# pgvector/pgvector

Hardware: AMD Instinct MI355X
Metric: QPS @ recall@10 (IVFFlat, 1M x 1536d) (higher is better)
Workload: dtype f32

## Files before the change

### pgvector_amd/csrc/kernels_query.hip

```cpp
#include "pgv_device.h"
#include "pgv_select.h"

#include <type_traits>

namespace pgv {

namespace {

constexpr int kQThreads = kSelThreads;
constexpr int kQWaves = kQThreads / kWave;
constexpr int kMaxBatchLists = 256;
constexpr int kHeadCap = 1024;

template <typename T, int METRIC, int NCH> struct WholeRows {
    Raw16 q[NCH];
    __device__ __forceinline__ void load_query(const char *qp, int lane) {
#pragma unroll
        for (int c = 0; c < NCH; c++) q[c] = load16(qp + ((size_t)c * kWave + lane) * sizeof(Raw16));
    }
    __device__ __forceinline__ float pair(const char *a, const char *b, int lane) const {
        Raw16 ra[NCH], rb[NCH];
#pragma unroll
        for (int c = 0; c < NCH; c++) ra[c] = load16(a + ((size_t)c * kWave + lane) * sizeof(Raw16));
#pragma unroll
// ... 727 lines not shown
    run_geometry(ctx, g, ix->nlists, &per, &grid);
    const int kp = pow2_at_least(max_probes);
    PGV_TRY(dispatch_metric(ix->metric, ix->dtype, [&](auto *tp, auto mc) {
        using T = std::remove_pointer_t<decltype(tp)>;
        constexpr int M = decltype(mc)::value;
        return dispatch_nch<T, M>(g, [&](auto nc) {
            constexpr int NCH = decltype(nc)::value;
            hipLaunchKernelGGL((mq_rank_kernel<T, M, NCH>), dim3(grid, nq), dim3(kQThreads), 0, ctx->stream,
                               static_cast<const char *>(ix->centers), ix->nlists, g.nvec, g.lpr_log2,
                               static_cast<const char *>(q_dev), cdist, cd_stride, per);
            PGV_HIP(hipGetLastError());
            return PGV_OK;
        });
    }));
    hipLaunchKernelGGL(mq_lists_kernel, dim3(nq), dim3(kQThreads), kQueryLds, ctx->stream, cdist, cd_stride, ix->nlists,
                       max_probes, kp, out_lists, out_dist);
    PGV_HIP(hipGetLastError());
    return PGV_OK;
}

int launch_multi_scan(pgv_ctx *ctx, const pgv_index *ix, const void *q_dev, int nq, const int32_t *probe_lists, int nprobes,
                      int64_t rows_bound, float *seg, int64_t seg_stride, int k, float *out_dist, int64_t *out_slot,
                      uint64_t *out_tid) {
    const RowGeom &g = ix->geom;
    int per, grid;
    run_geometry(ctx, g, rows_bound, &per, &grid);
    const int cap = (ctx->num_cus * 8 + nq - 1) / nq;
    if (grid > cap) grid = cap < 1 ? 1 : cap;
    PGV_TRY(dispatch_metric(ix->metric, ix->dtype, [&](auto *tp, auto mc) {
        using T = std::remove_pointer_t<decltype(tp)>;
        constexpr int M = decltype(mc)::value;
        return dispatch_nch<T, M>(g, [&](auto nc) {
            constexpr int NCH = decltype(nc)::value;
            hipLaunchKernelGGL((mq_scan_kernel<T, M, NCH>), dim3(grid, nq), dim3(kQThreads), 0, ctx->stream,
                               static_cast<const char *>(ix->vectors), ix->list_offsets, probe_lists, nprobes, g.nvec,
                               g.lpr_log2, static_cast<const char *>(q_dev), seg, seg_stride, per);
            PGV_HIP(hipGetLastError());
            return PGV_OK;
        });
    }));
    double *stats = (ctx->profiling && ctx->stats_dev.p) ? ctx->stats_dev.as<double>() : nullptr;
    hipLaunchKernelGGL(mq_head_kernel, dim3(nq), dim3(kQThreads), kQueryLds, ctx->stream, seg, seg_stride, ix->list_offsets,
                       ix->tids, probe_lists, nprobes, k, pow2_at_least(k), out_dist, out_slot, out_tid, stats);
    PGV_HIP(hipGetLastError());
    return PGV_OK;
}

namespace {
struct ApproxScratch {
    float *cand_val = nullptr;
    int64_t *cand_pos = nullptr;
    int32_t *flags = nullptr;
    int carve(DBuf &buf, int nq, int kprime) {
        const size_t nk = (size_t)nq * kprime;
        const size_t a1 = (sizeof(float) * nk + 15) & ~(size_t)15, a2 = a1 + sizeof(int64_t) * nk;
        PGV_TRY(buf.ensure(a2 + sizeof(int32_t) * (2 * (size_t)nq + 1)));
        cand_val = buf.as<float>();
        cand_pos = reinterpret_cast<int64_t *>(buf.as<char>() + a1);
        flags = reinterpret_cast<int32_t *>(buf.as<char>() + a2);
        return PGV_OK;
    }
};
}

int launch_exact_tail(pgv_ctx *ctx, const ExactTail &t, DBuf &scratch) {
    if (t.nq <= 0) return PGV_OK;
    const ExactRows &xr = t.rows;
    const bool dense = t.dense();
    if (dense ? (t.fixed_len <= 0 || t.probe_off || t.seg_start || t.probes != 0)
              : (t.fixed_len != 0 || !t.probe_off || !t.seg_start || t.probes < 1))
        PGV_FAIL(PGV_ERR_ARG, "exact tail: a list plan or one dense run");
    if (t.kprime > kRecheckCap || t.k > t.kprime)
        PGV_FAIL(PGV_ERR_ARG, "exact tail: k' = %d outside k..%d", t.kprime, kRecheckCap);
    if (t.pair_t && xr.dtype != PGV_F32) PGV_FAIL(PGV_ERR_ARG, "exact tail: pair terms are for fp32 rows");
    static_assert(kWide >= kRecheckCap, "k <= k' <= kWide: batch_fix_kernel's emit");
    if (t.emit.cnt && !(dense && t.pair_t && t.out_i32 && t.emit.probe_off && t.emit.seg_len && t.emit.list_off))
        PGV_FAIL(PGV_ERR_ARG, "exact tail: the plan is counted where the pair terms are written");
    ApproxScratch sc;
    PGV_TRY(sc.carve(scratch, t.nq, t.kprime));
    const int64_t *cand_slot = dense ? sc.cand_pos : nullptr;
    const int64_t *seg_start = dense ? nullptr : t.seg_start;
    const int64_t fixed_len = dense ? t.fixed_len : 0;
    PGV_TRY(launch_topk_segments(ctx, t.approx, seg_start, t.nq, fixed_len, t.kprime, sc.cand_val, sc.cand_pos,
                                 sc.flags + t.nq, t.emit.cnt, t.emit.cnt ? 2 * (int)fixed_len : 0));
#define PGV_RECHECK(T, DOT)                                                                                          \
    hipLaunchKernelGGL((batch_recheck_kernel<T, DOT>), dim3(t.nq), dim3(kQThreads), 0, ctx->stream,                   \
                       static_cast<const char *>(xr.vectors), xr.tids, xr.geom.nvec, xr.geom.lpr_log2,                \
                       static_cast<const char *>(t.queries), t.kprime, t.k, sc.cand_val, sc.cand_pos, cand_slot,      \
                       xr.list_offsets, t.probe_lists, t.probe_off, t.probes, seg_start, fixed_len, xr.norm_max,      \
                       t.bound, t.eps_add, t.nq, t.out_dist, t.out_slot, t.out_tid, t.out_i32, sc.flags, t.pair_t,    \
                       t.emit)
    if (t.pair_t)
        PGV_RECHECK(float, true);
    else if (xr.dtype == PGV_F32)
        PGV_RECHECK(float, false);
    else
        PGV_RECHECK(__half, false);
#undef PGV_RECHECK
    PGV_HIP(hipGetLastError());
    double *stats = (ctx->profiling && ctx->stats_dev.p) ? ctx->stats_dev.as<double>() : nullptr;
    int kp = 2;
    while (kp < t.k) kp <<= 1;
    const int cap = kp > kFastCap ? kp : kFastCap;
    const size_t lds = (size_t)cap * 8 + sizeof(SelShared);
    const int grid = t.nq < ctx->num_cus ? t.nq : ctx->num_cus;
#define PGV_FIX(T)                                                                                                    \
    hipLaunchKernelGGL(batch_fix_kernel<T>, dim3(grid), dim3(kQThreads), lds, ctx->stream,                            \
                       static_cast<const char *>(xr.vectors), xr.list_offsets, xr.tids, xr.geom.nvec,                 \
                       xr.geom.lpr_log2, static_cast<const char *>(t.queries), t.probe_lists, t.probe_off, t.probes,  \
                       seg_start, fixed_len, sc.flags, t.nq, t.approx, t.k, kp, cap, xr.norm_max, t.bound, t.eps_add, \
                       ctx->no_widen ? 0 : 1, t.out_dist, t.out_slot, t.out_tid, t.out_i32, stats, t.pair_t, t.emit)
    if (xr.dtype == PGV_F32)
        PGV_FIX(float);
    else
        PGV_FIX(__half);
#undef PGV_FIX
    PGV_HIP(hipGetLastError());
    return PGV_OK;
}

}
```

### pgvector_amd/csrc/kernels_select.hip

```cpp
#include "pgv_device.h"
#include "pgv_select.h"

namespace pgv {

namespace {


__global__ void plan_count_kernel(const int32_t *__restrict__ probe_lists,
                                  const int64_t *__restrict__ list_off, int nq, int probes,
                                  int *__restrict__ cnt, int64_t *__restrict__ probe_off,
                                  int64_t *__restrict__ seg_len) {
    const int q = blockIdx.x * blockDim.x + threadIdx.x;
    if (q >= nq) return;
    int64_t run = 0;
    for (int p = 0; p < probes; p++) {
        const int l = probe_lists[(size_t)q * probes + p];
        probe_off[(size_t)q * probes + p] = run;
        run += list_off[l + 1] - list_off[l];
        atomicAdd(&cnt[l], 1);
    }
    seg_len[q] = run;
}

template <typename F>
// ... 81 lines not shown
                                                const int64_t *__restrict__ seg_start,
                                                const int64_t *__restrict__ pair_start, int *__restrict__ fill,
                                                int nq, int probes, const float *__restrict__ pair_t,
                                                ScanPair *__restrict__ pairs) {
    if (i >= (int64_t)nq * probes) return;
    const int q = (int)(i / probes);
    const int l = probe_lists[i];
    const int64_t pos = pair_start[l] + atomicAdd(&fill[l], 1);
    ScanPair pr;
    pr.out_rel = seg_start[q] + probe_off[i] - list_off[l];
    pr.query = q;
    pr.pad = pair_t ? (int32_t)__float_as_uint(pair_t[i]) : 0;
    pairs[pos] = pr;
}

__global__ void plan_pairs_kernel(const int32_t *__restrict__ probe_lists,
                                  const int64_t *__restrict__ list_off,
                                  const int64_t *__restrict__ probe_off,
                                  const int64_t *__restrict__ seg_start,
                                  const int64_t *__restrict__ pair_start, int *__restrict__ fill,
                                  int nq, int probes, const float *__restrict__ pair_t,
                                  ScanPair *__restrict__ pairs) {
    plan_pairs_body((int64_t)blockIdx.x * blockDim.x + threadIdx.x, probe_lists, list_off, probe_off, seg_start, pair_start,
                    fill, nq, probes, pair_t, pairs);
}

__device__ __forceinline__ void plan_tasks_body(int64_t first, int64_t stride, const int *__restrict__ cnt,
                                                const int64_t *__restrict__ list_off,
                                                const int64_t *__restrict__ pair_start,
                                                const int64_t *__restrict__ task_start, int nlists, int qt,
                                                int rows_per_task, ScanTask *__restrict__ tasks) {
    const int64_t ntasks = task_start[nlists];
    for (int64_t t = first; t < ntasks; t += stride) {
        int lo = 0, hi = nlists - 1;
        while (lo < hi) {
            const int mid = (lo + hi + 1) >> 1;
            if (task_start[mid] <= t)
                lo = mid;
            else
                hi = mid - 1;
        }
        const int l = lo;
        const int64_t len = list_off[l + 1] - list_off[l];
        const int ng = (cnt[l] + qt - 1) / qt;
        const int64_t rel = t - task_start[l];
        const int c = (int)(rel / ng), g = (int)(rel % ng);
        ScanTask task;
        task.row0 = list_off[l] + (int64_t)c * rows_per_task;
        const int64_t left = len - (int64_t)c * rows_per_task;
        task.nrows = (int)(left < rows_per_task ? left : rows_per_task);
        task.pair0 = (int)(pair_start[l] + (int64_t)g * qt);
        const int pl = cnt[l] - g * qt;
        task.npairs = pl < qt ? pl : qt;
        task.pad = ng > 1 ? 1 : 0;
        tasks[t] = task;
    }
}

__global__ void plan_tasks_kernel(const int *__restrict__ cnt, const int64_t *__restrict__ list_off,
                                  const int64_t *__restrict__ pair_start,
                                  const int64_t *__restrict__ task_start, int nlists, int qt,
                                  int rows_per_task, ScanTask *__restrict__ tasks) {
    plan_tasks_body((int64_t)blockIdx.x * blockDim.x + threadIdx.x, (int64_t)gridDim.x * blockDim.x, cnt, list_off,
                    pair_start, task_start, nlists, qt, rows_per_task, tasks);
}

__global__ void plan_pairs_tasks_kernel(const int32_t *__restrict__ probe_lists, const int64_t *__restrict__ list_off,
                                        const int64_t *__restrict__ probe_off, const int64_t *__restrict__ seg_start,
                                        const int64_t *__restrict__ pair_start, const int64_t *__restrict__ task_start,
                                        const int *__restrict__ cnt, int *__restrict__ fill, int nq, int probes, int nlists,
                                        int qt, int rows_per_task, const float *__restrict__ pair_t, int pair_blocks,
                                        ScanPair *__restrict__ pairs, ScanTask *__restrict__ tasks) {
    if ((int)blockIdx.x < pair_blocks)
        plan_pairs_body((int64_t)blockIdx.x * blockDim.x + threadIdx.x, probe_lists, list_off, probe_off, seg_start,
                        pair_start, fill, nq, probes, pair_t, pairs);
    else
        plan_tasks_body((int64_t)(blockIdx.x - pair_blocks) * blockDim.x + threadIdx.x,
                        (int64_t)(gridDim.x - pair_blocks) * blockDim.x, cnt, list_off, pair_start, task_start, nlists, qt,
                        rows_per_task, tasks);
}

__device__ __forceinline__ bool dist_before(float a, float b) { return float_to_key(a) < float_to_key(b); }


__global__ __launch_bounds__(kSelThreads) void topk_kernel(
    const float *__restrict__ vals, const int64_t *__restrict__ seg_start, int64_t fixed_len,
    int k, int kp, int cap, float *__restrict__ out_val, int64_t *__restrict__ out_pos,
    int32_t *__restrict__ zero_word, int32_t *__restrict__ zero_range, int zero_n) {
    extern __shared__ __attribute__((aligned(16))) char smem[];
    unsigned long long *ent = reinterpret_cast<unsigned long long *>(smem);
    SelShared *s = reinterpret_cast<SelShared *>(smem + (size_t)cap * 8);

    const int seg = blockIdx.x;
    if (zero_word && seg == 0 && threadIdx.x == 0) *zero_word = 0;
    if (zero_range)
        for (int i = seg * kSelThreads + (int)threadIdx.x; i < zero_n; i += (int)gridDim.x * kSelThreads) zero_range[i] = 0;
    const int64_t base = seg_start ? seg_start[seg] : (int64_t)seg * fixed_len;
    const int64_t m = seg_start ? seg_start[seg + 1] - base : fixed_len;
    const float *v = vals + base;
    block_topk_auto(v, m, k, kp, cap, ent, s);

    for (int i = threadIdx.x; i < k; i += kSelThreads) {
        const unsigned long long e = ent[i];
        const bool have = e != ~0ull && (int64_t)i < (m < k ? m : (int64_t)k);
        out_val[(size_t)seg * k + i] = have ? key_to_float((unsigned)(e >> 32)) : INFINITY;
        out_pos[(size_t)seg * k + i] = have ? (int64_t)(unsigned)(e & 0xffffffffu) : -1;
    }
}

__global__ void positions_to_slots_kernel(const int32_t *__restrict__ probe_lists,
                                          const int64_t *__restrict__ probe_off,
                                          const int64_t *__restrict__ list_off,
                                          const uint64_t *__restrict__ tids, int nq, int probes,
                                          int k, const int64_t *__restrict__ pos,
                                          int64_t *__restrict__ out_slot,
                                          uint64_t *__restrict__ out_tid) {
    const int64_t i = (int64_t)blockIdx.x * blockDim.x + threadIdx.x;
    if (i >= (int64_t)nq * k) return;
    const int q = (int)(i / k);
    const int64_t p = pos[i];
    int64_t slot = -1;
    if (p >= 0) {
        const int64_t *off = probe_off + (size_t)q * probes;
        int lo = 0, hi = probes - 1;
        while (lo < hi) {
            const int mid = (lo + hi + 1) >> 1;
            if (off[mid] <= p)
                lo = mid;
            else
                hi = mid - 1;
        }
        const int l = probe_lists[(size_t)q * probes + lo];
        slot = list_off[l] + (p - off[lo]);
    }
    if (out_slot) out_slot[i] = slot;
    if (out_tid) out_tid[i] = (slot >= 0 && tids) ? tids[slot] : ~0ull;
}

__global__ void iota_slots_kernel(const int32_t *__restrict__ lists,
                                  const int64_t *__restrict__ probe_off,
                                  const int64_t *__restrict__ list_off,
                                  int64_t *__restrict__ out_slot) {
    const int p = blockIdx.x;
    const int l = lists[p];
    const int64_t beg = list_off[l], len = list_off[l + 1] - beg;
    for (int64_t i = threadIdx.x; i < len; i += blockDim.x) out_slot[probe_off[p] + i] = beg + i;
}

__global__ __launch_bounds__(256) void plan_stats_kernel(const int *__restrict__ cnt,
                                                         const int64_t *__restrict__ list_off,
                                                         const int64_t *__restrict__ totals, int nlists,
                                                         int qt, double *__restrict__ acc) {
    __shared__ double red[256], red_u[256];
    double rows = 0.0, uniq = 0.0;
    for (int l = threadIdx.x; l < nlists; l += 256) {
        const double len = (double)(list_off[l + 1] - list_off[l]);
        rows += (double)((cnt[l] + qt - 1) / qt) * len;
        uniq += cnt[l] > 0 ? len : 0.0;
    }
    red[threadIdx.x] = rows;
    red_u[threadIdx.x] = uniq;
    __syncthreads();
    for (int s = 128; s > 0; s >>= 1) {
        if (threadIdx.x < s) {
            red[threadIdx.x] += red[threadIdx.x + s];
            red_u[threadIdx.x] += red_u[threadIdx.x + s];
        }
        __syncthreads();
    }
    if (threadIdx.x == 0) {
        acc[0] += (double)totals[0];
        acc[1] += red[0];
        acc[5] += red_u[0];
    }
}

__global__ void merge_heads_kernel(const float *__restrict__ dist_all, const uint64_t *__restrict__ tid_all, int nranks,
                                   int nq, int k, float *__restrict__ out_dist, uint64_t *__restrict__ out_tid) {
    const int q = blockIdx.x * blockDim.x + threadIdx.x;
    if (q >= nq) return;
    int at[16];
    for (int r = 0; r < nranks; r++) at[r] = 0;
    for (int i = 0; i < k; i++) {
// ... 49 lines not shown
    pb->probe_off = ctx->plan_b.as<int64_t>();
    pb->seg_len = pb->probe_off + npairs;
    pb->seg_start = pb->seg_len + nq;
    pb->pair_start = pb->seg_start + nq + 1;
    pb->task_start = pb->pair_start + nlists + 1;
    pb->totals = pb->task_start + nlists + 1;
    return PGV_OK;
}

int launch_plan_batch(pgv_ctx *ctx, const pgv_index *ix, const int32_t *probe_lists, int nq,
                      int probes, int qt, int rows_per_task, bool read_totals, PlanResult *res, const float *pair_t,
                      bool counted) {
    const int nlists = ix->nlists;
    const size_t npairs = (size_t)nq * probes;

    int64_t max_chunks = 0, sum_chunks = 0;
    for (int l = 0; l < nlists; l++) {
        const int64_t nc = (ix->h_offsets[l + 1] - ix->h_offsets[l] + rows_per_task - 1) / rows_per_task;
        sum_chunks += nc;
        if (nc > max_chunks) max_chunks = nc;
    }
    res->ntasks_bound = max_chunks * (int64_t)(npairs / qt) + sum_chunks;
    res->out_bound = (int64_t)nq * ix->len_prefix[probes];
    if (res->ntasks_bound > 0x7fffffff) PGV_FAIL(PGV_ERR_ARG, "plan: too many tasks");

    PlanBuffers pb;
    PGV_TRY(plan_batch_reserve(ctx, nlists, nq, probes, &pb));
    PGV_TRY(ctx->pairs.ensure(sizeof(ScanPair) * npairs));
    PGV_TRY(ctx->tasks.ensure(sizeof(ScanTask) * (size_t)(res->ntasks_bound > 0 ? res->ntasks_bound : 1) + 16));
    int *cnt = pb.cnt, *fill = pb.fill;
    int64_t *probe_off = pb.probe_off, *seg_len = pb.seg_len, *seg_start = pb.seg_start, *pair_start = pb.pair_start;
    int64_t *task_start = pb.task_start, *totals = pb.totals;
    ScanTask *tasks = ctx->tasks.as<ScanTask>();
    const int64_t want = (res->ntasks_bound + 255) / 256;
    const int64_t cap = (int64_t)ctx->num_cus * 8;
    const unsigned task_blocks = (unsigned)(want < 1 ? 1 : (want > cap ? cap : want));
    const unsigned pair_blocks = (unsigned)((npairs + 255) / 256);
    res->ntasks = res->ntasks_bound;
    res->total_out = res->out_bound;

    if (counted) {
        double *acc = nullptr;
        if (read_totals) {
            PGV_TRY(ctx->stats_dev.ensure(8 * sizeof(double)));
            acc = ctx->stats_dev.as<double>();
        }
        hipLaunchKernelGGL(plan_scan_kernel, dim3(1), dim3(1024), 0, ctx->stream, cnt, ix->list_offsets, seg_len, nq, nlists,
                           qt, rows_per_task, seg_start, pair_start, task_start, totals, acc);
        hipLaunchKernelGGL(plan_pairs_tasks_kernel, dim3(pair_blocks + task_blocks), dim3(256), 0, ctx->stream, probe_lists,
                           ix->list_offsets, probe_off, seg_start, pair_start, task_start, cnt, fill, nq, probes, nlists, qt,
                           rows_per_task, pair_t, (int)pair_blocks, ctx->pairs.as<ScanPair>(), tasks);
        PGV_HIP(hipGetLastError());
    } else {
        PGV_HIP(hipMemsetAsync(cnt, 0, sizeof(int) * 2 * (size_t)nlists, ctx->stream));
        hipLaunchKernelGGL(plan_count_kernel, dim3((nq + 255) / 256), dim3(256), 0, ctx->stream,
                           probe_lists, ix->list_offsets, nq, probes, cnt, probe_off, seg_len);
        hipLaunchKernelGGL(plan_scan_kernel, dim3(1), dim3(1024), 0, ctx->stream, cnt,
                           ix->list_offsets, seg_len, nq, nlists, qt, rows_per_task, seg_start,
                           pair_start, task_start, totals, static_cast<double *>(nullptr));
        hipLaunchKernelGGL(plan_pairs_kernel, dim3(pair_blocks), dim3(256), 0,
                           ctx->stream, probe_lists, ix->list_offsets, probe_off, seg_start,
                           pair_start, fill, nq, probes, pair_t, ctx->pairs.as<ScanPair>());
        hipLaunchKernelGGL(plan_tasks_kernel, dim3(task_blocks), dim3(256), 0,
                           ctx->stream, cnt, ix->list_offsets, pair_start, task_start, nlists, qt, rows_per_task, tasks);
        PGV_HIP(hipGetLastError());
        if (read_totals) {
            PGV_TRY(ctx->stats_dev.ensure(8 * sizeof(double)));
            hipLaunchKernelGGL(plan_stats_kernel, dim3(1), dim3(256), 0, ctx->stream, cnt,
                               ix->list_offsets, totals, nlists, qt, ctx->stats_dev.as<double>());
            PGV_HIP(hipGetLastError());
        }
    }
    res->tasks = tasks;
    res->pairs = ctx->pairs.as<ScanPair>();
    res->ntasks_dev = reinterpret_cast<int *>(totals + 2);
    res->seg_start = seg_start;
    res->probe_off = probe_off;
    res->pair_start = pair_start;
    return PGV_OK;
}

int launch_topk_segments(pgv_ctx *ctx, const float *vals, const int64_t *seg_start, int nseg,
                         int64_t fixed_len, int k, float *out_val, int64_t *out_pos, int32_t *zero_word,
                         int32_t *zero_range, int zero_n) {
    if (nseg <= 0 || k <= 0) return PGV_OK;
    if (k > 4096) PGV_FAIL(PGV_ERR_ARG, "top-k: k = %d exceeds the supported 4096", k);
    int kp = 1;
    while (kp < k) kp <<= 1;
    if (kp < 2) kp = 2;
    const int cap = kp > kFastCap ? kp : kFastCap;
    const size_t lds = (size_t)cap * 8 + sizeof(SelShared);
    hipLaunchKernelGGL(topk_kernel, dim3(nseg), dim3(kSelThreads), lds, ctx->stream, vals,
                       seg_start, fixed_len, k, kp, cap, out_val, out_pos, zero_word, zero_range, zero_n);
    PGV_HIP(hipGetLastError());
    return PGV_OK;
}

int launch_positions_to_slots(pgv_ctx *ctx, const pgv_index *ix, const int32_t *probe_lists,
                              const int64_t *probe_off, int nq, int probes, int k,
                              const int64_t *pos, int64_t *out_slot, uint64_t *out_tid) {
    const int64_t total = (int64_t)nq * k;
    if (total <= 0) return PGV_OK;
    hipLaunchKernelGGL(positions_to_slots_kernel, dim3((unsigned)((total + 255) / 256)), dim3(256),
                       0, ctx->stream, probe_lists, probe_off, ix->list_offsets, ix->tids, nq,
                       probes, k, pos, out_slot, out_tid);
    PGV_HIP(hipGetLastError());
    return PGV_OK;
}

int launch_iota_slots(pgv_ctx *ctx, const pgv_index *ix, const int32_t *lists_dev, int nlists,
                      const int64_t *probe_off, int64_t *out_slot) {
    if (nlists <= 0) return PGV_OK;
    hipLaunchKernelGGL(iota_slots_kernel, dim3(nlists), dim3(256), 0, ctx->stream, lists_dev,
                       probe_off, ix->list_offsets, out_slot);
    PGV_HIP(hipGetLastError());
    return PGV_OK;
}

}
```

### pgvector_amd/csrc/pgv_abi_ivf.hip

```cpp
#include "pgv_abi_common.h"

extern "C" {


namespace {
struct IndexLayout {
    size_t centers, vectors, offsets, tids, row_norms, center_norms, bytes;
    bool has_tids, has_norms;
};
IndexLayout index_layout(int nlists, int64_t n, size_t row_bytes, bool has_tids, bool l2) {
    auto up = [](size_t v) { return (v + 255) & ~(size_t)255; };
    IndexLayout L{};
    size_t at = 0;
    L.centers = at; at = up(at + (size_t)nlists * row_bytes);
    L.vectors = at; at = up(at + (size_t)(n > 0 ? n : 1) * row_bytes);
    L.offsets = at; at = up(at + sizeof(int64_t) * ((size_t)nlists + 1));
    L.has_tids = has_tids;
    L.tids = at; if (has_tids) at = up(at + sizeof(uint64_t) * (size_t)n);
    L.has_norms = l2;
    L.row_norms = at; if (l2 && n > 0) at = up(at + sizeof(float) * ((size_t)n + 1));
    L.center_norms = at; if (l2) at = up(at + sizeof(float) * ((size_t)nlists + 1));
    L.bytes = at;
    return L;
}
// ... 908 lines not shown
static int list_scan_step(pgv_index *ix, const ScanPath &path, const ScanWork &work, const void *queries, const float *qscale,
                          double counted, float *out) {
    pgv_ctx *ctx = ix->ctx;
    const RowsView v = path.shadow ? ivf_shadow_rows(ix) : ivf_rows(ix);
    PGV_TRY(scan_turn_begin(ctx));
    ScanTimer timer{ctx};
    PGV_TRY(timer.begin(counted, counted));
    if (path.bits)
        PGV_TRY(launch_hamming_lists(ctx, v, queries, bit_query_bytes(ix->nbits), work, path.qt, out));
    else if (path.use_mfma)
        PGV_TRY(launch_mfma_scan(ctx, v, queries, work, ix->row_norms, nullptr, out, rows_stream_past_caches(v), path.qt,
                                 path.shadow ? qscale : nullptr));
    else if (path.use_tile)
        PGV_TRY(launch_tile_scan(ctx, v, queries, work, out));
    else
        PGV_TRY(launch_scan(ctx, v, queries, work, path.qt, out));
    PGV_TRY(timer.end());
    return scan_turn_end(ctx);
}

static int scan_batch_impl(pgv_index *ix, const void *q_dev, int nq, const int32_t *probe_lists, int probes,
                           int k, float *out_dist, int64_t *out_slot, uint64_t *out_tid, ShadowBatch *sb) {
    pgv_ctx *ctx = ix->ctx;
    const ScanPath path = scan_path(ix, nq, probes, k);
    if (path.per_query) {
        const int64_t bound = ix->len_prefix[probes];
        const int64_t seg_stride = (bound + 7) / 4 * 4;
        PGV_TRY(ctx->plan_d.ensure(sizeof(float) * (size_t)nq * seg_stride));
        OutArg od, os, ot;
        PGV_TRY(od.init(out_dist, sizeof(float) * (size_t)nq * k, ctx->out_stage));
        PGV_TRY(os.init(out_slot, sizeof(int64_t) * (size_t)nq * k, ctx->out_stage2));
        PGV_TRY(ot.init(out_tid, sizeof(uint64_t) * (size_t)nq * k, ctx->sel_b));
        PGV_TRY(scan_turn_begin(ctx));
        ScanTimer timer{ctx};
        PGV_TRY(timer.begin(0.0, 0.0));
        PGV_TRY(launch_multi_scan(ctx, ix, q_dev, nq, probe_lists, probes, bound, ctx->plan_d.as<float>(), seg_stride, k,
                                  od.as<float>(), os.as<int64_t>(), ot.as<uint64_t>()));
        PGV_TRY(timer.end());
        PGV_TRY(scan_turn_end(ctx));
        bool need = false;
        PGV_TRY(od.finish(ctx, &need));
        PGV_TRY(os.finish(ctx, &need));
        PGV_TRY(ot.finish(ctx, &need));
        return sync_if(ctx, need);
    }
    ShadowBatch own;
    if (!sb) sb = &own;
    if (path.shadow && !sb->cast_for_scan) PGV_TRY(shadow_batch_cast(ix, q_dev, nq, probes, false, true, sb));
    const float *pair_t = (path.shadow && sb->pairs_done) ? sb->pair_t : nullptr;
    PlanResult plan;
    PGV_TRY(launch_plan_batch(ctx, ix, probe_lists, nq, probes, path.qt, path.rows_per_task, ctx->profiling, &plan, pair_t,
                              pair_t != nullptr));
    if (path.shadow) {
        if (!pair_t)
            PGV_TRY(launch_shadow_pairs(ctx, ix->geom, q_dev, ix->centers, plan.pair_start, ix->nlists, (int64_t)nq * probes,
                                        plan.pairs));
        ctx->scan_shadow_queries += nq;
    }

    PGV_TRY(ctx->plan_d.ensure(sizeof(float) * (size_t)(plan.out_bound > 0 ? plan.out_bound : 1)));
    float *seg_vals = ctx->plan_d.as<float>();
    if (plan.ntasks_bound > 0)
        PGV_TRY(list_scan_step(ix, path, plan.work(), path.shadow ? sb->qcast : q_dev, sb->qscale, 0.0, seg_vals));

    OutArg od, os, ot;
    PGV_TRY(od.init(out_dist, sizeof(float) * (size_t)nq * k, ctx->out_stage));
    PGV_TRY(os.init(out_slot, sizeof(int64_t) * (size_t)nq * k, ctx->out_stage2));
    PGV_TRY(ot.init(out_tid, sizeof(uint64_t) * (size_t)nq * k, ctx->sel_b));
    PGV_TRY(ctx->sel_a.ensure(sizeof(int64_t) * (size_t)nq * k));
    int64_t *pos = ctx->sel_a.as<int64_t>();
    if (path.approx) {
        ExactTail tail;
        tail.rows = {ix->vectors, ix->tids, ix->list_offsets, ix->geom, ix->dtype,
                     reinterpret_cast<const unsigned *>(ix->row_norms + ix->nrows)};
        tail.queries = q_dev;
        tail.nq = nq;
        tail.kprime = approx_candidates(k);
        tail.k = k;
        tail.approx = seg_vals;
        tail.probe_lists = probe_lists;
        tail.probe_off = plan.probe_off;
        tail.probes = probes;
        tail.seg_start = plan.seg_start;
        tail.bound = scan_bound_chain(ctx, ix->geom.ld, scan_chain_length(ix->geom, ix->dtype, path.wide));
        if (path.shadow) tail.bound = shadow_band(ix->geom.ld, tail.bound.g_ref);
        tail.eps_add = path.shadow ? sb->qeps : nullptr;
        tail.out_dist = od.as<float>();
        tail.out_slot = os.as<int64_t>();
        tail.out_tid = ot.as<uint64_t>();
        PGV_TRY(launch_exact_tail(ctx, tail, ctx->ms_a));
    } else {
        PGV_TRY(launch_topk_segments(ctx, seg_vals, plan.seg_start, nq, 0, k, od.as<float>(), pos));
        PGV_TRY(launch_positions_to_slots(ctx, ix, probe_lists, plan.probe_off, nq, probes, k, pos,
                                          os.as<int64_t>(), ot.as<uint64_t>()));
    }
    bool need = false;
    PGV_TRY(od.finish(ctx, &need));
    PGV_TRY(os.finish(ctx, &need));
    PGV_TRY(ot.finish(ctx, &need));
    return sync_if(ctx, need);
}

int scan_batch_dev(pgv_index *ix, const void *q_dev, int nq, const int32_t *probe_lists, int probes, int k, float *out_dist,
                   int64_t *out_slot, uint64_t *out_tid) {
    return scan_batch_impl(ix, q_dev, nq, probe_lists, probes, k, out_dist, out_slot, out_tid, nullptr);
}

int pgv_scan_lists(pgv_index *ix, const void *query, const int32_t *lists, int nlists,
                   float *out_dist, int64_t *out_slot, int64_t capacity, int64_t *out_count) {
    if (!ix || !out_count) PGV_FAIL(PGV_ERR_ARG, "pgv_scan_lists: index/out_count is NULL");
    if (nlists < 0 || (nlists > 0 && !lists)) PGV_FAIL(PGV_ERR_ARG, "bad list array");
    pgv_ctx *ctx = ix->ctx;
    PGV_HIP(hipSetDevice(ctx->device));

    std::vector<int32_t> hl((size_t)nlists);
    if (nlists) {
        if (is_device_ptr(lists))
            PGV_HIP(hipMemcpy(hl.data(), lists, sizeof(int32_t) * (size_t)nlists, hipMemcpyDeviceToHost));
        else
            memcpy(hl.data(), lists, sizeof(int32_t) * (size_t)nlists);
    }
    int64_t m = 0;
    for (int p = 0; p < nlists; p++) {
        if (hl[p] < 0 || hl[p] >= ix->nlists) PGV_FAIL(PGV_ERR_ARG, "list id %d out of range", hl[p]);
        m += ix->h_offsets[hl[p] + 1] - ix->h_offsets[hl[p]];
    }
    *out_count = m;
    if (m > capacity) PGV_FAIL(PGV_ERR_ARG, "output capacity %lld < %lld tuples", (long long)capacity, (long long)m);
    if (m == 0) return PGV_OK;
    if (!out_dist || !out_slot) PGV_FAIL(PGV_ERR_ARG, "out_dist/out_slot is NULL");

    OutArg od, os;
    PGV_TRY(od.init(out_dist, sizeof(float) * (size_t)m, ctx->out_stage));
    PGV_TRY(os.init(out_slot, sizeof(int64_t) * (size_t)m, ctx->out_stage2));

    ScanPath path;
    path.bits = ix->nbits > 0;
    path.qt = path.bits ? hamming_list_group_size(1.0) : 1;
    path.rows_per_task = path.bits ? hamming_list_rows_per_task() : rows_per_task_for(ctx, m, 1);
    const int ch = path.rows_per_task;
    int64_t ntasks = 0;
    for (int p = 0; p < nlists; p++) {
        int64_t len = ix->h_offsets[hl[p] + 1] - ix->h_offsets[hl[p]];
        ntasks += (len + ch - 1) / ch;
    }
    const size_t tb = sizeof(ScanTask) * (size_t)ntasks, pb = sizeof(ScanPair) * (size_t)nlists,
                 ob = sizeof(int64_t) * (size_t)nlists, lb = sizeof(int32_t) * (size_t)nlists;
    PGV_TRY(staging_acquire(ctx));
    PGV_TRY(ctx->h_a.ensure(tb + pb + ob + lb + 16));
    char *hb = ctx->h_a.as<char>();
    ScanTask *ht = reinterpret_cast<ScanTask *>(hb);
    ScanPair *hp = reinterpret_cast<ScanPair *>(hb + tb);
    int64_t *hoff = reinterpret_cast<int64_t *>(hb + tb + pb);
    int32_t *hlist = reinterpret_cast<int32_t *>(hb + tb + pb + ob);
    int *hn = reinterpret_cast<int *>(hb + tb + pb + ob + lb);
    int64_t t = 0, run = 0;
    for (int p = 0; p < nlists; p++) {
        const int64_t beg = ix->h_offsets[hl[p]], len = ix->h_offsets[hl[p] + 1] - beg;
        hp[p].out_rel = run - beg;
        hp[p].query = 0;
        hp[p].pad = 0;
        hoff[p] = run;
        hlist[p] = hl[p];
        for (int64_t c = 0; c * ch < len; c++) {
            ht[t].row0 = beg + c * ch;
            int64_t left = len - c * ch;
            ht[t].nrows = (int)(left < ch ? left : ch);
            ht[t].pair0 = p;
            ht[t].npairs = 1;
            ht[t].pad = 0;
            t++;
        }
        run += len;
    }
    *hn = (int)ntasks;
// ... 304 lines not shown
```

### pgvector_amd/csrc/pgv_internal.h

```cpp
#pragma once

#include <hip/hip_runtime.h>

#include <cstdint>
#include <cstdio>
#include <cstdlib>
#include <cstring>
#include <cmath>
#include <vector>

#include "../../include/pgv_hip.h"

namespace pgv {

void set_error(const char *fmt, ...) __attribute__((format(printf, 1, 2)));

#define PGV_FAIL(code, ...)            \
    do {                               \
        ::pgv::set_error(__VA_ARGS__); \
        return (code);                 \
    } while (0)

#define PGV_HIP(call)                                                                  \
    do {                                                                               \
// ... 386 lines not shown
                           int *list_rec, int *nrec, int32_t *rec_owner, int32_t *rec_lc, int32_t *rec_list,
                           const int64_t *rec_off, int *rec_fill, int32_t *link_elem, float *link_dist);
int launch_hnsw_link_size(pgv_ctx *ctx, const HnswGraph &graph, const uint8_t *nb_flag, const int32_t *rec_owner,
                          const int32_t *rec_lc, const int32_t *rec_list, const int *list_count, int64_t *rec_off, int nrec,
                          int pass, int64_t *rec_pos, int32_t *rec_nstart, int32_t *rec_from, const int32_t *rec_wait,
                          int64_t *size_ids, int64_t *size_pairs);
int launch_hnsw_link_scan(pgv_ctx *ctx, int64_t *a, int64_t *b, int64_t *c, int n, int64_t *totals);
int launch_hnsw_link_stats(pgv_ctx *ctx, const int *blocked, const int64_t *totals, int64_t *stats);
int launch_hnsw_link_pairs(pgv_ctx *ctx, const int32_t *nbr, const int64_t *rec_pos, const int32_t *rec_nstart,
                           const int32_t *rec_from, const int64_t *rec_off, int32_t *link_elem, float *link_dist,
                           const int32_t *rec_list, int *list_count, int nrec, int pass,
                           const int64_t *ids_start, int32_t *ids, const int64_t *pair_start, int32_t *a, int32_t *b);
int launch_hnsw_link_replay(pgv_ctx *ctx, const HnswGraph &graph, float *nb_dist, uint8_t *nb_flag, int nrec, int pass,
                            const int32_t *rec_lc, const int64_t *rec_off, const float *link_dist, const int64_t *rec_pos,
                            const int32_t *rec_nstart, const int32_t *rec_from, const int64_t *ids_start, const int32_t *ids,
                            const int64_t *pair_start, const float *tri, const int64_t *mm_start, const float *mm,
                            int32_t *rec_wait, int16_t *loc_save, int *blocked);
int launch_hnsw_link_new(pgv_ctx *ctx, const HnswGraph &graph, float *nb_dist, uint8_t *nb_flag, const int32_t *elems,
                         const uint8_t *linked, int nq, int lcap, const int32_t *sel_ids, const float *sel_dist,
                         const uint8_t *sel_closer, const int32_t *sel_cnt);
bool mfma_argmin_supported(int mode, int64_t n, int k);
int launch_argmin_mfma(pgv_ctx *ctx, int mode, pgv_dtype dtype, const RowGeom &g, const void *rows, int64_t n,
                       const void *centers, int k, int32_t *out_idx, float *out_val);

int mfma_scan_rows_per_task();
int mfma_scan_queries_per_task();
int launch_mfma_dense(pgv_ctx *ctx, pgv_metric metric, pgv_dtype dtype, const RowGeom &g, const void *rows, int64_t n,
                      const void *queries, int nq, const float *row_norms, float *out, int64_t out_stride);
int dense_chain_length(const RowGeom &g, pgv_dtype dtype);
int launch_row_norms(pgv_ctx *ctx, const RowsView &v, float *out, unsigned *max_bits);
int launch_mfma_scan(pgv_ctx *ctx, const RowsView &v, const void *queries, const ScanWork &w, const float *row_norms,
                     const float *query_norms, float *out, bool stream_rows, int queries_per_task = 32,
                     const float *shadow_scale = nullptr);
int launch_shadow_build(pgv_ctx *ctx, const RowGeom &g32, const RowGeom &g16, const void *rows, const void *centers,
                        const int64_t *list_off, int nlists, int64_t n, void *shadow, void *words);
int shadow_scale_of(float max_abs);
int shadow_chain_length(const RowGeom &g16);
int scan_chain_length(const RowGeom &g, pgv_dtype dtype, bool wide);
int launch_shadow_query(pgv_ctx *ctx, const RowGeom &g32, const RowGeom &g16, const void *queries, int nq,
                        const ShadowTerms &st, const RankShadowTerms &rt, const float *center_norm_max,
                        const float *row_norm_max, void *qcast, float *qscale, float *qeps, float *cscale, float *ceps);
int launch_shadow_pairs(pgv_ctx *ctx, const RowGeom &g32, const void *queries, const void *centers,
                        const int64_t *pair_start, int nlists, int64_t npairs, ScanPair *pairs);
int mfma_scan_queries_per_task_wide();

int launch_gather_words(pgv_ctx *ctx, const void *src, int words_per_row, int64_t nrows, const int64_t *idx, int n,
                        uint32_t *out);
size_t build_sort_scratch_bytes(int64_t n, int key_bits);
int launch_build_order(pgv_ctx *ctx, const int32_t *lists, int64_t n, int nlists, unsigned long long *keys_tmp,
                       unsigned long long *keys_sorted, unsigned long long *counts, int64_t *offsets, int *bad,
                       void *sort_scratch, size_t sort_scratch_bytes);
int launch_build_gather(pgv_ctx *ctx, const void *src_rows, const unsigned long long *keys_sorted, int64_t n, int nvec,
                        void *dst_rows, const uint64_t *src_tids, uint64_t *dst_tids);

struct PlanResult {
    ScanTask *tasks = nullptr;
    ScanPair *pairs = nullptr;
    int *ntasks_dev = nullptr;
    int64_t ntasks = 0;
    int64_t total_out = 0;
    int64_t ntasks_bound = 0;
    int64_t out_bound = 0;
    int64_t *seg_start = nullptr;
    int64_t *probe_off = nullptr;
    int64_t *pair_start = nullptr;
    ScanWork work() const { return {tasks, ntasks_dev, (int)ntasks_bound, pairs}; }
};
struct PlanBuffers {
    int *cnt = nullptr, *fill = nullptr;
    int64_t *probe_off = nullptr, *seg_len = nullptr;
    int64_t *seg_start = nullptr, *pair_start = nullptr, *task_start = nullptr, *totals = nullptr;
};
int plan_batch_reserve(pgv_ctx *ctx, int nlists, int nq, int probes, PlanBuffers *pb);
struct PlanEmit {
    int *cnt = nullptr;
    int64_t *probe_off = nullptr, *seg_len = nullptr;
    const int64_t *list_off = nullptr;
};
int launch_plan_batch(pgv_ctx *ctx, const pgv_index *ix, const int32_t *probe_lists, int nq,
                      int probes, int qt, int rows_per_task, bool read_totals, PlanResult *res,
                      const float *pair_t = nullptr, bool counted = false);
int launch_topk_segments(pgv_ctx *ctx, const float *vals, const int64_t *seg_start, int nseg,
                         int64_t fixed_len, int k, float *out_val, int64_t *out_pos, int32_t *zero_word = nullptr,
                         int32_t *zero_range = nullptr, int zero_n = 0);
int launch_positions_to_slots(pgv_ctx *ctx, const pgv_index *ix, const int32_t *probe_lists,
                              const int64_t *probe_off, int nq, int probes, int k,
                              const int64_t *pos, int64_t *out_slot, uint64_t *out_tid);
struct ExactRows {
    const void *vectors;
    const uint64_t *tids;
    const int64_t *list_offsets;
    pgv::RowGeom geom;
    pgv_dtype dtype;
    const unsigned *norm_max;
};
struct ExactTail {
    ExactRows rows;
    const void *queries = nullptr;
    int nq = 0;
    int kprime = 0;
    int k = 0;
    float *approx = nullptr;
    const int32_t *probe_lists = nullptr;
    const int64_t *probe_off = nullptr;
    int probes = 0;
    const int64_t *seg_start = nullptr;
    int64_t fixed_len = 0;
    ScanBound bound{};
    const float *eps_add = nullptr;
    float *out_dist = nullptr;
    int64_t *out_slot = nullptr;
    uint64_t *out_tid = nullptr;
    int32_t *out_i32 = nullptr;
    float *pair_t = nullptr;
    PlanEmit emit;
    bool dense() const { return probe_lists == nullptr; }
};
int launch_exact_tail(pgv_ctx *ctx, const ExactTail &t, DBuf &scratch);
int launch_iota_slots(pgv_ctx *ctx, const pgv_index *ix, const int32_t *lists_dev, int nlists,
                      const int64_t *probe_off, int64_t *out_slot);

int query_max_batch_lists();
int query_head_cap();
size_t query_head_bytes(int head);
int launch_query_stage(pgv_ctx *ctx, const void *src_pinned, void *dst_dev, int nvec);
int launch_multi_rank(pgv_ctx *ctx, const pgv_index *ix, const void *q_dev, int nq, float *cdist, int64_t cd_stride,
                      int max_probes, int32_t *out_lists, float *out_dist);
int launch_multi_scan(pgv_ctx *ctx, const pgv_index *ix, const void *q_dev, int nq, const int32_t *probe_lists, int nprobes,
                      int64_t rows_bound, float *seg, int64_t seg_stride, int k, float *out_dist, int64_t *out_slot,
                      uint64_t *out_tid);
int launch_query_iota(pgv_ctx *ctx, int32_t *out, int n);
int launch_one_query_rows(pgv_ctx *ctx, const RowsView &v, const void *q_dev, float *out);
int launch_query_rank(pgv_ctx *ctx, const pgv_index *ix, const void *q_dev, float *cdist, int max_probes,
                      int32_t *out_lists);
int launch_query_scan(pgv_ctx *ctx, const pgv_index *ix, const void *q_dev, const int32_t *probe_lists, int nprobes,
                      int64_t rows_bound, float *seg);
int launch_query_head(pgv_ctx *ctx, const pgv_index *ix, const float *seg, const int32_t *probe_lists, int nprobes,
                      int skip, int count, void *head_rec, unsigned seq);

int launch_merge_heads(pgv_ctx *ctx, const float *dist_all, const uint64_t *tid_all, int nranks, int nq, int k,
                       float *out_dist, uint64_t *out_tid);

int launch_cast_pos_to_i32(pgv_ctx *ctx, const int64_t *pos, int64_t n, int32_t *out);

int kmpp_block_count(int n);
int launch_kmpp_update(pgv_ctx *ctx, const float *raw, float *weight, int n, int spherical,
                       double *block_sums);
int launch_kmpp_pick(pgv_ctx *ctx, const RowGeom &g, const void *samples, int n,
                     const float *weight, const double *block_sums, const double *draws,
                     int round, void *centers, int32_t *picked);
int launch_kmpp_total(pgv_ctx *ctx, const double *block_sums, int nblocks, double *out);
int launch_kmpp_pick_sharded(pgv_ctx *ctx, const RowGeom &g, const void *samples, int n, const float *weight,
                             const double *block_sums, const double *totals, const int64_t *counts, int nranks, int rank,
                             const double *draws, int round, void *send_row, int32_t *owner_out);
int launch_kmpp_take_row(pgv_ctx *ctx, const RowGeom &g, const void *gathered, const int32_t *owner, void *centers,
                         int round);
int launch_lloyd_pack(pgv_ctx *ctx, const int32_t *counts, const unsigned long long *changes, int k, float *tail);
int launch_lloyd_unpack(pgv_ctx *ctx, const float *tail, int k, int32_t *counts, unsigned long long *changes,
                        long long *host_rec, long long seq);
int launch_changes_hist(pgv_ctx *ctx, const int32_t *closest_new, int32_t *closest_io, int n,
                        int32_t *counts, unsigned long long *changes);
int launch_members(pgv_ctx *ctx, const int32_t *closest, int n, int k, const int32_t *counts,
                   int32_t *offsets, int32_t *members);
int launch_center_sums(pgv_ctx *ctx, pgv_dtype dtype, const RowGeom &g, const void *samples,
                       const int32_t *offsets, const int32_t *members, int k, float *sums);
int launch_finish_centers(pgv_ctx *ctx, pgv_dtype dtype, const RowGeom &g, int k, int dim,
                          const float *sums, const int32_t *counts, const float *refill,
                          const int32_t *refill_row, void *centers);
int launch_normalize_rows(pgv_ctx *ctx, pgv_dtype dtype, const RowGeom &g, void *rows, int64_t n,
                          int dim, int32_t *flag);
int launch_check_centers(pgv_ctx *ctx, pgv_dtype dtype, const RowGeom &g, const void *centers,
                         int k, int dim, int check_zero_norm, int32_t *flag);

}
```

### pgvector_amd/csrc/pgv_select.h

```cpp
#pragma once

#include "pgv_device.h"


namespace pgv {

namespace {

constexpr int kSelThreads = 256;
constexpr int kBins = 2048;
constexpr int kFastCap = 1024;

struct SelShared {
    unsigned hist[kBins];
    unsigned scan[kSelThreads];
    unsigned wave_tot[kSelThreads / kWave];
    unsigned count;
    unsigned bin;
    unsigned remaining;
    unsigned running;
};

__device__ inline void pick_bin(SelShared *s, int nbins, unsigned want) {
    const int per = nbins / kSelThreads;
// ... 137 lines not shown
            __syncthreads();
            for (int i = threadIdx.x; i < cap; i += kSelThreads) ent[i] = ~0ull;
            if (threadIdx.x == 0) s->count = 0;
            __syncthreads();
        }
    }

    if (done) {
    } else if (m <= k) {
        for (int64_t i = threadIdx.x; i < m; i += kSelThreads)
            ent[i] = ((unsigned long long)float_to_key(load(i)) << 32) | (unsigned)i;
        __syncthreads();
    } else {
        unsigned prefix = 0;
        unsigned want = (unsigned)(k - 1);
        unsigned count_eq = 0;
        for (int pass = 0; pass < 3; pass++) {
            const int shift = pass == 0 ? 21 : (pass == 1 ? 10 : 0);
            const int nbins = pass == 2 ? 1024 : 2048;
            for (int i = threadIdx.x; i < kBins; i += kSelThreads) s->hist[i] = 0;
            __syncthreads();
            for (int64_t i = threadIdx.x; i < m; i += kSelThreads) {
                const unsigned key = float_to_key(load(i));
                const bool in = pass == 0 || (pass == 1 ? (key >> 21) == (prefix >> 21)
                                                        : (key >> 10) == (prefix >> 10));
                if (in) atomicAdd(&s->hist[(key >> shift) & (nbins - 1)], 1u);
            }
            __syncthreads();
            pick_bin(s, nbins, want);
            prefix |= s->bin << shift;
            want = s->remaining;
            count_eq = s->hist[s->bin];
            __syncthreads();
        }
        const unsigned thr = prefix;
        const unsigned need_eq = want + 1;
        if (threadIdx.x == 0) s->running = 0;
        __syncthreads();
        const bool ordered = count_eq > need_eq;
        const int64_t padded = (m + kSelThreads - 1) / kSelThreads * kSelThreads;
        for (int64_t i = threadIdx.x; i < padded; i += kSelThreads) {
            const unsigned key = i < m ? float_to_key(load(i)) : 0xffffffffu;
            const bool valid = i < m;
            if (valid && key < thr) {
                const unsigned at = atomicAdd(&s->count, 1u);
                ent[at] = ((unsigned long long)key << 32) | (unsigned)i;
            }
            if (!ordered) {
                if (valid && key == thr) {
                    const unsigned at = atomicAdd(&s->count, 1u);
                    ent[at] = ((unsigned long long)key << 32) | (unsigned)i;
                }
            } else {
                const bool eq = valid && key == thr;
                const unsigned long long bal = __ballot(eq);
                const int lane = threadIdx.x & (kWave - 1), wave = threadIdx.x >> 6;
                const unsigned before_lane = __popcll(bal & ((1ull << lane) - 1ull));
                if (lane == 0) s->wave_tot[wave] = (unsigned)__popcll(bal);
                __syncthreads();
                unsigned before_wave = 0, tile_tot = 0;
                for (int w = 0; w < kSelThreads / kWave; w++) {
                    if (w < wave) before_wave += s->wave_tot[w];
                    tile_tot += s->wave_tot[w];
                }
                const unsigned rank = s->running + before_wave + before_lane;
                if (eq && rank < need_eq) {
                    const unsigned at = atomicAdd(&s->count, 1u);
                    ent[at] = ((unsigned long long)key << 32) | (unsigned)i;
                }
                __syncthreads();
                if (threadIdx.x == 0) s->running += tile_tot;
                __syncthreads();
            }
        }
        __syncthreads();
    }

    sort_entries(ent, sort_n);
}

constexpr int kSmallVec = 12;
constexpr int kLargeVec = 20;
constexpr int kSmallMax = kLargeVec * 4 * kSelThreads;
constexpr int kExtractMax = 16;

template <int NVEC>
__device__ __forceinline__ bool block_topk_small(const float *v, int m, int skip, int k, int kp, int cap,
                                                 unsigned long long *ent, SelShared *s) {
    for (int i = threadIdx.x; i < cap; i += kSelThreads) ent[i] = ~0ull;
    if (threadIdx.x == 0) s->count = 0;
    const int last4 = ((m + 3) & ~3) - 4;
    float4 r[NVEC];
#pragma unroll
    for (int b = 0; b < NVEC; b++) {
        const int at = b * 4 * kSelThreads + 4 * (int)threadIdx.x;
        r[b] = *reinterpret_cast<const float4 *>(v + (at < last4 ? at : last4));
    }
    float fmine = INFINITY;
#pragma unroll
    for (int b = 0; b < NVEC; b++) {
        const int at = b * 4 * kSelThreads + 4 * (int)threadIdx.x;
        if (at + 3 >= m) {
            if (at + 0 >= m) r[b].x = INFINITY;
            if (at + 1 >= m) r[b].y = INFINITY;
            if (at + 2 >= m) r[b].z = INFINITY;
            if (at + 3 >= m) r[b].w = INFINITY;
        }
        if (b == 0 && at == 0) {
            if (skip > 0) r[b].x = INFINITY;
            if (skip > 1) r[b].y = INFINITY;
            if (skip > 2) r[b].z = INFINITY;
        }
        fmine = fminf(fminf(fmine, fminf(r[b].x, r[b].y)), fminf(r[b].z, r[b].w));
    }
    const unsigned key_mine = float_to_key(fmine);
    const unsigned comp = (key_mine & ~0xffu) | threadIdx.x;
    unsigned *mins = s->hist;
    if (k <= kExtractMax) {
        const int lane = threadIdx.x & (kWave - 1), wave = threadIdx.x >> 6;
        unsigned v = comp, keep = 0xffffffffu;
#pragma unroll 1
        for (int j = 0; j < k; j++) {
            const unsigned mn = wave_min_u32(v);
            keep = lane == j ? mn : keep;
            v = v == mn ? 0xffffffffu : v;
        }
        const int n4 = (kSelThreads / kWave) * k;
        __syncthreads();
        if (lane < k) mins[wave * k + lane] = keep;
        if ((int)threadIdx.x >= n4 && (int)threadIdx.x < ((n4 + 3) & ~3)) mins[threadIdx.x] = 0xffffffffu;
        __syncthreads();
        if ((int)threadIdx.x < n4) {
            const unsigned own = mins[threadIdx.x];
            const uint4 *m4 = reinterpret_cast<const uint4 *>(mins);
            unsigned rank = 0;
            for (int j4 = 0; j4 < (n4 + 3) / 4; j4++) {
                const uint4 o = m4[j4];
                rank += (o.x < own) + (o.y < own) + (o.z < own) + (o.w < own);
            }
            if (rank == (unsigned)(k - 1)) s->bin = own | 0xffu;
        }
    } else {
        __syncthreads();
        mins[threadIdx.x] = comp;
        __syncthreads();
        unsigned rank = 0;
        {
            const uint4 *m4 = reinterpret_cast<const uint4 *>(mins);
#pragma unroll 4
            for (int j4 = 0; j4 < kSelThreads / 4; j4++) {
                const uint4 o = m4[j4];
                rank += (o.x < comp) + (o.y < comp) + (o.z < comp) + (o.w < comp);
            }
        }
        if (rank == (unsigned)(k - 1)) s->bin = key_mine | 0xffu;
    }
    __syncthreads();
    const unsigned t0 = s->bin;
    const bool general = t0 >= float_to_key(INFINITY);
    if (!general) {
        const float t0f = key_to_float(t0);
        unsigned cnt = 0;
#pragma unroll
        for (int b = 0; b < NVEC; b++)
            cnt += (r[b].x <= t0f) + (r[b].y <= t0f) + (r[b].z <= t0f) + (r[b].w <= t0f);
        if (cnt) {
            unsigned slot = atomicAdd(&s->count, cnt);
#pragma unroll
            for (int b = 0; b < NVEC; b++) {
                const int at = b * 4 * kSelThreads + 4 * (int)threadIdx.x;
                const float e[4] = {r[b].x, r[b].y, r[b].z, r[b].w};
                if (fminf(fminf(e[0], e[1]), fminf(e[2], e[3])) <= t0f) {
#pragma unroll
                    for (int c = 0; c < 4; c++)
                        if (e[c] <= t0f) {
                            if (slot < (unsigned)cap)
                                ent[slot] = ((unsigned long long)float_to_key(e[c]) << 32) | (unsigned)(at + c - skip);
                            slot++;
                        }
                }
            }
        }
    }
    __syncthreads();
    const unsigned got = s->count;
    if (!general && got <= (unsigned)kSelThreads) {
        rank_sort_entries(ent, (int)got);
    } else if (!general && got <= (unsigned)cap) {
        int sort_n = kp;
        while (sort_n < (int)got) sort_n <<= 1;
        sort_entries(ent, sort_n);
    } else {
        __syncthreads();
        return false;
    }
    return true;
}

__device__ __forceinline__ void block_topk_auto(const float *v, int64_t m, int k, int kp, int cap, unsigned long long *ent,
                                                SelShared *s) {
    bool done = false;
    const int skip = (int)((reinterpret_cast<uintptr_t>(v) >> 2) & 3);
    const int64_t ma = m + skip;
    if (m > k && ma <= kSmallMax && k <= kSelThreads / 2) {
        const float *va = v - skip;
        if (ma <= 4 * kSelThreads)
            done = block_topk_small<1>(va, (int)ma, skip, k, kp, cap, ent, s);
        else if (ma <= 16 * kSelThreads)
            done = block_topk_small<4>(va, (int)ma, skip, k, kp, cap, ent, s);
        else if (ma <= kSmallVec * 4 * kSelThreads)
            done = block_topk_small<kSmallVec>(va, (int)ma, skip, k, kp, cap, ent, s);
        else
            done = block_topk_small<kLargeVec>(va, (int)ma, skip, k, kp, cap, ent, s);
    }
    if (!done) block_topk([v](int64_t i) { return v[i]; }, m, k, kp, cap, ent, s);
}

}

}
```

Measured before the change: 1.374 million.

## Specialize top-k kernel by segment length class and add register-tail path for long segments

The top-k kernel is templated on a length class chosen on the host from a bound on segment length, so short-segment launches compile only the small register paths, with lower register pressure. A new long-segment variant of block_topk_small streams extra tail chunks from memory and records survivors in a 64-bit mask. This lets segments up to a larger size avoid the general radix-select fallback. The cost is re-reading tail data from global memory two or three times, plus extra template instantiations. The host bound comes from the list length prefix at the probe count.

```diff
diff --git a/pgvector_amd/csrc/kernels_query.hip b/pgvector_amd/csrc/kernels_query.hip
--- a/pgvector_amd/csrc/kernels_query.hip
+++ b/pgvector_amd/csrc/kernels_query.hip
@@ -833,7 +833,8 @@
     const int64_t *seg_start = dense ? nullptr : t.seg_start;
     const int64_t fixed_len = dense ? t.fixed_len : 0;
     PGV_TRY(launch_topk_segments(ctx, t.approx, seg_start, t.nq, fixed_len, t.kprime, sc.cand_val, sc.cand_pos,
-                                 sc.flags + t.nq, t.emit.cnt, t.emit.cnt ? 2 * (int)fixed_len : 0));
+                                 sc.flags + t.nq, t.emit.cnt, t.emit.cnt ? 2 * (int)fixed_len : 0,
+                                 dense ? 0 : t.seg_bound));
 #define PGV_RECHECK(T, DOT)                                                                                          \
     hipLaunchKernelGGL((batch_recheck_kernel<T, DOT>), dim3(t.nq), dim3(kQThreads), 0, ctx->stream,                   \
                        static_cast<const char *>(xr.vectors), xr.tids, xr.geom.nvec, xr.geom.lpr_log2,                \
diff --git a/pgvector_amd/csrc/kernels_select.hip b/pgvector_amd/csrc/kernels_select.hip
--- a/pgvector_amd/csrc/kernels_select.hip
+++ b/pgvector_amd/csrc/kernels_select.hip
@@ -187,7 +187,29 @@
 
 __device__ __forceinline__ bool dist_before(float a, float b) { return float_to_key(a) < float_to_key(b); }
 
-
+enum TopkClass { kTopkSmall = 0, kTopkMedium = 1, kTopkLong = 2 };
+constexpr int kLongVec = 16;
+constexpr int kLongTail = 16;
+constexpr int kLongMax = (kLongVec + kLongTail) * 4 * kSelThreads;
+
+template <int CLS>
+__device__ __forceinline__ bool topk_class_forms(const float *va, int ma, int skip, int k, int kp, int cap,
+                                                 unsigned long long *ent, SelShared *s) {
+    if constexpr (CLS == kTopkSmall) {
+        if (ma <= 4 * kSelThreads) return block_topk_small<1>(va, ma, skip, k, kp, cap, ent, s);
+    } else if constexpr (CLS == kTopkMedium) {
+        if (ma <= 4 * kSelThreads) return block_topk_small<1>(va, ma, skip, k, kp, cap, ent, s);
+        if (ma <= 16 * kSelThreads) return block_topk_small<4>(va, ma, skip, k, kp, cap, ent, s);
+    } else {
+        if (ma <= 16 * kSelThreads) return block_topk_small<4>(va, ma, skip, k, kp, cap, ent, s);
+        if (ma <= kSmallVec * 4 * kSelThreads) return block_topk_small<kSmallVec>(va, ma, skip, k, kp, cap, ent, s);
+        if (ma <= kLongVec * 4 * kSelThreads) return block_topk_small<kLongVec>(va, ma, skip, k, kp, cap, ent, s);
+        if (ma <= kLongMax) return block_topk_small<kLongVec, kLongTail>(va, ma, skip, k, kp, cap, ent, s);
+    }
+    return false;
+}
+
+template <int CLS>
 __global__ __launch_bounds__(kSelThreads) void topk_kernel(
     const float *__restrict__ vals, const int64_t *__restrict__ seg_start, int64_t fixed_len,
     int k, int kp, int cap, float *__restrict__ out_val, int64_t *__restrict__ out_pos,
@@ -203,7 +225,12 @@
     const int64_t base = seg_start ? seg_start[seg] : (int64_t)seg * fixed_len;
     const int64_t m = seg_start ? seg_start[seg + 1] - base : fixed_len;
     const float *v = vals + base;
-    block_topk_auto(v, m, k, kp, cap, ent, s);
+    bool done = false;
+    const int skip = (int)((reinterpret_cast<uintptr_t>(v) >> 2) & 3);
+    const int64_t ma = m + skip;
+    if (m > k && ma <= kLongMax && k <= kSelThreads / 2)
+        done = topk_class_forms<CLS>(v - skip, (int)ma, skip, k, kp, cap, ent, s);
+    if (!done) block_topk([v](int64_t i) { return v[i]; }, m, k, kp, cap, ent, s);
 
     for (int i = threadIdx.x; i < k; i += kSelThreads) {
         const unsigned long long e = ent[i];
@@ -419,7 +446,7 @@
 
 int launch_topk_segments(pgv_ctx *ctx, const float *vals, const int64_t *seg_start, int nseg,
                          int64_t fixed_len, int k, float *out_val, int64_t *out_pos, int32_t *zero_word,
-                         int32_t *zero_range, int zero_n) {
+                         int32_t *zero_range, int zero_n, int64_t len_bound) {
     if (nseg <= 0 || k <= 0) return PGV_OK;
     if (k > 4096) PGV_FAIL(PGV_ERR_ARG, "top-k: k = %d exceeds the supported 4096", k);
     int kp = 1;
@@ -427,8 +454,18 @@
     if (kp < 2) kp = 2;
     const int cap = kp > kFastCap ? kp : kFastCap;
     const size_t lds = (size_t)cap * 8 + sizeof(SelShared);
-    hipLaunchKernelGGL(topk_kernel, dim3(nseg), dim3(kSelThreads), lds, ctx->stream, vals,
-                       seg_start, fixed_len, k, kp, cap, out_val, out_pos, zero_word, zero_range, zero_n);
+    int64_t ma_bound = 0;
+    if (!seg_start)
+        ma_bound = fixed_len + (fixed_len % 4 == 0 ? (int64_t)((reinterpret_cast<uintptr_t>(vals) >> 2) & 3) : 3);
+    else if (len_bound > 0)
+        ma_bound = len_bound + 3;
+    auto kernel = topk_kernel<kTopkLong>;
+    if (ma_bound > 0 && ma_bound <= 4 * kSelThreads)
+        kernel = topk_kernel<kTopkSmall>;
+    else if (ma_bound > 0 && ma_bound <= 16 * kSelThreads)
+        kernel = topk_kernel<kTopkMedium>;
+    hipLaunchKernelGGL(kernel, dim3(nseg), dim3(kSelThreads), lds, ctx->stream, vals, seg_start, fixed_len, k, kp, cap,
+                       out_val, out_pos, zero_word, zero_range, zero_n);
     PGV_HIP(hipGetLastError());
     return PGV_OK;
 }
diff --git a/pgvector_amd/csrc/pgv_abi_ivf.hip b/pgvector_amd/csrc/pgv_abi_ivf.hip
--- a/pgvector_amd/csrc/pgv_abi_ivf.hip
+++ b/pgvector_amd/csrc/pgv_abi_ivf.hip
@@ -1014,6 +1014,7 @@
         tail.probe_off = plan.probe_off;
         tail.probes = probes;
         tail.seg_start = plan.seg_start;
+        tail.seg_bound = ix->len_prefix[probes];
         tail.bound = scan_bound_chain(ctx, ix->geom.ld, scan_chain_length(ix->geom, ix->dtype, path.wide));
         if (path.shadow) tail.bound = shadow_band(ix->geom.ld, tail.bound.g_ref);
         tail.eps_add = path.shadow ? sb->qeps : nullptr;
@@ -1022,7 +1023,8 @@
         tail.out_tid = ot.as<uint64_t>();
         PGV_TRY(launch_exact_tail(ctx, tail, ctx->ms_a));
     } else {
-        PGV_TRY(launch_topk_segments(ctx, seg_vals, plan.seg_start, nq, 0, k, od.as<float>(), pos));
+        PGV_TRY(launch_topk_segments(ctx, seg_vals, plan.seg_start, nq, 0, k, od.as<float>(), pos, nullptr, nullptr, 0,
+                                     ix->len_prefix[probes]));
         PGV_TRY(launch_positions_to_slots(ctx, ix, probe_lists, plan.probe_off, nq, probes, k, pos,
                                           os.as<int64_t>(), ot.as<uint64_t>()));
     }
diff --git a/pgvector_amd/csrc/pgv_internal.h b/pgvector_amd/csrc/pgv_internal.h
--- a/pgvector_amd/csrc/pgv_internal.h
+++ b/pgvector_amd/csrc/pgv_internal.h
@@ -492,7 +492,7 @@
                       const float *pair_t = nullptr, bool counted = false);
 int launch_topk_segments(pgv_ctx *ctx, const float *vals, const int64_t *seg_start, int nseg,
                          int64_t fixed_len, int k, float *out_val, int64_t *out_pos, int32_t *zero_word = nullptr,
-                         int32_t *zero_range = nullptr, int zero_n = 0);
+                         int32_t *zero_range = nullptr, int zero_n = 0, int64_t len_bound = 0);
 int launch_positions_to_slots(pgv_ctx *ctx, const pgv_index *ix, const int32_t *probe_lists,
                               const int64_t *probe_off, int nq, int probes, int k,
                               const int64_t *pos, int64_t *out_slot, uint64_t *out_tid);
@@ -515,6 +515,7 @@
     const int64_t *probe_off = nullptr;
     int probes = 0;
     const int64_t *seg_start = nullptr;
+    int64_t seg_bound = 0;
     int64_t fixed_len = 0;
     ScanBound bound{};
     const float *eps_add = nullptr;
diff --git a/pgvector_amd/csrc/pgv_select.h b/pgvector_amd/csrc/pgv_select.h
--- a/pgvector_amd/csrc/pgv_select.h
+++ b/pgvector_amd/csrc/pgv_select.h
@@ -243,9 +243,10 @@
 constexpr int kSmallVec = 12;
 constexpr int kLargeVec = 20;
 constexpr int kSmallMax = kLargeVec * 4 * kSelThreads;
+constexpr int kTailGroup = 2;
 constexpr int kExtractMax = 16;
 
-template <int NVEC>
+template <int NVEC, int NTAIL = 0>
 __device__ __forceinline__ bool block_topk_small(const float *v, int m, int skip, int k, int kp, int cap,
                                                  unsigned long long *ent, SelShared *s) {
     for (int i = threadIdx.x; i < cap; i += kSelThreads) ent[i] = ~0ull;
@@ -257,7 +258,30 @@
         const int at = b * 4 * kSelThreads + 4 * (int)threadIdx.x;
         r[b] = *reinterpret_cast<const float4 *>(v + (at < last4 ? at : last4));
     }
+    auto tail_at = [](int j) { return (NVEC + j) * 4 * kSelThreads + 4 * (int)threadIdx.x; };
+    auto tail_load = [&](int j) {
+        const int at = tail_at(j);
+        float4 t = *reinterpret_cast<const float4 *>(v + (at < last4 ? at : last4));
+        if (at + 0 >= m) t.x = INFINITY;
+        if (at + 1 >= m) t.y = INFINITY;
+        if (at + 2 >= m) t.z = INFINITY;
+        if (at + 3 >= m) t.w = INFINITY;
+        return t;
+    };
+    (void)tail_load;
     float fmine = INFINITY;
+    const int ntail = NTAIL > 0 ? (m - NVEC * 4 * kSelThreads + 4 * kSelThreads - 1) / (4 * kSelThreads) : 0;
+    if constexpr (NTAIL > 0) {
+        static_assert(NTAIL % kTailGroup == 0 && NTAIL <= 16, "whole groups; one bit of a 64-bit mask per tail value");
+#pragma unroll 1
+        for (int j0 = 0; j0 < ntail; j0 += kTailGroup) {
+            float4 t[kTailGroup];
+#pragma unroll
+            for (int j = 0; j < kTailGroup; j++) t[j] = tail_load(j0 + j);
+#pragma unroll
+            for (int j = 0; j < kTailGroup; j++) fmine = fminf(fminf(fmine, fminf(t[j].x, t[j].y)), fminf(t[j].z, t[j].w));
+        }
+    }
 #pragma unroll
     for (int b = 0; b < NVEC; b++) {
         const int at = b * 4 * kSelThreads + 4 * (int)threadIdx.x;
@@ -322,11 +346,46 @@
     if (!general) {
         const float t0f = key_to_float(t0);
         unsigned cnt = 0;
-#pragma unroll
-        for (int b = 0; b < NVEC; b++)
+        unsigned long long tail_mask = 0;
+        if constexpr (NTAIL > 0) {
+#pragma unroll 1
+            for (int j0 = 0; j0 < ntail; j0 += kTailGroup) {
+                float4 t[kTailGroup];
+#pragma unroll
+                for (int j = 0; j < kTailGroup; j++) t[j] = tail_load(j0 + j);
+#pragma unroll
+                for (int j = 0; j < kTailGroup; j++)
+                    tail_mask |= (unsigned long long)((t[j].x <= t0f ? 1u : 0u) | (t[j].y <= t0f ? 2u : 0u) |
+                                                      (t[j].z <= t0f ? 4u : 0u) | (t[j].w <= t0f ? 8u : 0u))
+                                 << (4 * (j0 + j));
+            }
+            cnt = __popcll(tail_mask);
+        }
+#pragma unroll
+        for (int b = 0; b < NVEC; b++) {
             cnt += (r[b].x <= t0f) + (r[b].y <= t0f) + (r[b].z <= t0f) + (r[b].w <= t0f);
+            if constexpr (NTAIL > 0) asm volatile("" : "+v"(cnt));
+        }
         if (cnt) {
             unsigned slot = atomicAdd(&s->count, cnt);
+            if constexpr (NTAIL > 0) {
+#pragma unroll 1
+                for (unsigned long long left = tail_mask; left;) {
+                    const int j = (__ffsll(left) - 1) >> 2;
+                    const unsigned bits = (unsigned)(left >> (4 * j)) & 15u;
+                    left &= ~(15ull << (4 * j));
+                    const int at = tail_at(j);
+                    const float4 t = *reinterpret_cast<const float4 *>(v + (at < last4 ? at : last4));
+                    const float e[4] = {t.x, t.y, t.z, t.w};
+#pragma unroll
+                    for (int c = 0; c < 4; c++)
+                        if (bits & (1u << c)) {
+                            if (slot < (unsigned)cap)
+                                ent[slot] = ((unsigned long long)float_to_key(e[c]) << 32) | (unsigned)(at + c - skip);
+                            slot++;
+                        }
+                }
+            }
 #pragma unroll
             for (int b = 0; b < NVEC; b++) {
                 const int at = b * 4 * kSelThreads + 4 * (int)threadIdx.x;
```

After: 1.402 million, median of 6. 2.0% higher.
